# athas/raytracers

Hardware: AMD Instinct MI355X
Metric: Mray/s (primary+secondary) on rgbbox & irreg 1000x1000 (higher is better)
Workload: dtype f32

## Files before the change

raytracers_amd/csrc/api.cpp:

```cpp
#include <hip/hip_runtime.h>

#include <algorithm>
#include <chrono>
#include <cmath>
#include <cstdio>
#include <cstdlib>
#include <cstring>
#include <memory>
#include <string>
#include <vector>

#include "../../include/rt_mi355x.h"
#include "rt_device.hpp"
#include "rt_host.hpp"
#include "rt_internal.hpp"

namespace rti {
int fail(rt_context *ctx, const std::string &msg) {
  if (ctx) ctx->err = msg;
  return 1;
}
int hip_fail(rt_context *ctx, hipError_t e, const char *what) {
  return fail(ctx, std::string(what) + ": " + hipGetErrorString(e));
}
// ... 388 lines not shown
bool rt_scene_exceeds_l2(const rt_prepared *ps) { return static_cast<int64_t>(ps->n) * 80 > (int64_t(32) << 20); }

void set_cull(const rt_context *ctx, const rt_prepared *ps, const Plan &pl, const float *cams_dev, rtk::KParams *p) {
  if (ctx->cull == 0 || !ps->cull.ok || pl.variant != RT_VARIANT_POOLED || (pl.waves != 16 && pl.waves != 4)) return;
  if (ctx->cull < 0 && pl.lds_nodes == p->n_nodes && pl.lds_sph == p->n_sph) return;
  if (cams_dev == nullptr ? !rt::cull_origin_ok(ps->cull, &p->cam.ox) : (cams_dev != ctx->cams_dev || ctx->cams_host == nullptr)) return;
  for (int f = 0; cams_dev != nullptr && f < p->nframes; ++f)
    if (!rt::cull_origin_ok(ps->cull, ctx->cams_host + 12 * f)) return;
  p->cull = 1;
  p->cull_c2 = ps->cull.c2;
  p->cull_kappa = ps->cull.kappa;
}

void set_dark(const rt_context *ctx, bool instrumented, rtk::KParams *p) {
  p->dark = (ctx->dark_stop != 0 && p->cost == nullptr && (!instrumented || ctx->dark_stop > 0)) ? 1 : 0;
}

std::string pooled_launch_name(const rtk::KParams &p, int waves, int rays = 0) {
  rtk::PooledKey k{};
  return rtk::choose_pooled(p, false, waves, rays, &k) ? rtk::pooled_name(k) : "none";
}
const char *pooled_launch_nodes(const rtk::KParams &p, int waves) {
  rtk::PooledKey k{};
  return rtk::choose_pooled(p, false, waves, 0, &k) && rtk::pooled_presort(k) ? "sign-ordered" : "planes";
}

void frame_params(const rt_prepared *ps, int64_t h, int64_t w, int rows_per_tile, int part, int nparts, int max_depth, const float *cam12, rtk::KParams *p) {
  scene_params(ps, p);
  std::memcpy(&p->cam, cam12 ? static_cast<const void *>(cam12) : static_cast<const void *>(&ps->cam), sizeof(p->cam));
  p->w = static_cast<int>(w); p->h = static_cast<int>(h);
// ... 349 lines not shown
    RT_HIP(ctx, rtk::launch_persistent(p, false, pl.grid, pl.waves, ctx->stream));
    ctx->last_launch = "family=persistent";
    return 0;
  }
  if (ps->n >= (int64_t(1) << 22)) return fail(ctx, "pooled kernel: at most 2^22 spheres (work items and hit keys carry the leaf index in 22 bits)");
  if (p.rpt_log2 < 0) return fail(ctx, "pooled kernel: rows_per_tile must be a power of two");
  if (int rc = get_uv(ctx, w, h, &p.u_tab, &p.v_tab)) return rc;
  tick("uv tables");
  TileOrder *to = nullptr;
  if (ctx->adaptive_order && !p.cams)
    if (int rc = find_view(ctx, ps, p, pl, &to)) return rc;
  Tickets t;
  if (int rc = choose_tickets(ctx, ps, to, xq, tick, p, pl, &t)) return rc;
  set_cull(ctx, ps, pl, cams_dev, &p);
  set_dark(ctx, false, &p);
  tick("before launch");
  RT_HIP(ctx, rtk::launch_pooled(p, false, pl.grid, pl.waves, ctx->stream));
  tick("launch_pooled");
  char buf[256];
  std::snprintf(buf, sizeof buf, "family=pooled tickets=%s%s instantiation=%s frames=%d tiles=%d grid=%d waves=%d counters=%d%s deep_class=%d deep_split=%d recording=%d nodes=%s,dark=%d",
                p.px_hdr ? "pixel-list" : t.first_order ? "tiles-bit-reversed" : (p.order ? "tiles-ordered" : "tiles-raster"), t.borrowed ? "(borrowed)" : "",
                pooled_launch_name(p, pl.waves).c_str(), p.nframes, p.nchunks, pl.grid, pl.waves, p.nshards, p.interleave ? "(turns)" : "", p.px_hdr ? 0 : p.deep_class,
                p.px_hdr ? 0 : p.deep_split, p.cost ? (p.cost_px ? 2 : 1) : 0, pooled_launch_nodes(p, pl.waves), p.dark);
  ctx->last_launch = buf;
  if (to && p.cost) {
    to->sort_pending = true;
    to->sort_px = p.cost_px != nullptr;
    to->rec_out_skip = p.out_skip;
    if (ctx->eager_sort && (stream_was_idle || ctx->sync_policy))
      if (int rc = sort_view(ctx, ps, to, p, pl)) return rc;
    tick("record: eager sorts");
  }
  return 0;
}
using rti::enqueue_render;

extern "C" void rt_context_destroy(rt_context *ctx);

// ... 221 lines not shown
    ctx->px_solo_div = std::max(1, std::min(4096, v));
  } else if (k == "eager_sort") {
    drain_streams(ctx);
    ctx->eager_sort = v != 0;
  } else if (k == "borrow") {
    ctx->borrow = std::max(0, std::min(4, v));
  } else if (k == "stack_cap") {
    if (v != 0 && v != rtk::kSpillCapbTest) return fail(ctx, "stack_cap must be 0 or 192");
    ctx->stack_cap = v;
  } else if (k == "wide_waves") {
    ctx->wide_waves = std::max(0, std::min(2, v));
  } else if (k == "cull") {
    ctx->cull = std::max(-1, std::min(1, v));
  } else if (k == "dark_stop") {
    ctx->dark_stop = std::max(-1, std::min(1, v));
  } else if (k == "sync_policy") {
    ctx->sync_policy = v != 0;
  } else {
    return fail(ctx, "unknown option: " + k);
  }
  return 0;
}

extern "C" int rt_context_device_info(const rt_context *ctx, int *device, int *num_cu, int *lds_bytes, char *name,
                                      int name_len) {
  RT_LOCK(const_cast<rt_context *>(ctx));
  if (!ctx) return 1;
  if (device) *device = ctx->device;
  if (num_cu) *num_cu = ctx->num_cu;
  if (lds_bytes) *lds_bytes = ctx->lds_bytes;
// ... 66 lines not shown
  ps->bmax = reinterpret_cast<float *>(b + o_bmax); ps->left = reinterpret_cast<int32_t *>(b + o_left);
  ps->right = reinterpret_cast<int32_t *>(b + o_right); ps->parent = reinterpret_cast<int32_t *>(b + o_parent);
  ps->nodes = reinterpret_cast<float4 *>(b + o_nodes); ps->nodes64 = reinterpret_cast<float4 *>(b + o_nodes64);
  ps->sph = reinterpret_cast<float4 *>(b + o_sph); ps->col = reinterpret_cast<float4 *>(b + o_col);
  ps->ids = reinterpret_cast<int32_t *>(b + o_ids);
  return hipSuccess;
}

int host_build_upload(rt_context *ctx, rt_prepared *ps, const std::vector<rt::Sphere> &spheres, hipError_t *e) {
  const size_t n = spheres.size(), ni = n - 1;
  int rc = 0;
  auto put = [&](void *dst, const void *src, size_t bytes) {
    if (!rc && hipMemcpyAsync(dst, src, bytes, hipMemcpyHostToDevice, ctx->stream) != hipSuccess) rc = fail(ctx, "hipMemcpyAsync failed");
  };
  const rt::Lbvh bvh = rt::build_lbvh(spheres);
  const rt::TravLayout tl = rt::make_trav_layout(bvh, ctx->treelet);
  ps->height = tl.height;
  ps->tl_depth = tl.treelet_depth;
  put(ps->L7, bvh.L.data(), n * sizeof(rt::Sphere));
  put(ps->bmin, bvh.bmin.data(), ni * 3 * sizeof(float));
  put(ps->bmax, bvh.bmax.data(), ni * 3 * sizeof(float));
  put(ps->left, bvh.left.data(), ni * sizeof(int32_t));
  put(ps->right, bvh.right.data(), ni * sizeof(int32_t));
  put(ps->parent, bvh.parent.data(), ni * sizeof(int32_t));
  put(ps->nodes, tl.nodes.data(), ni * sizeof(rt::TravNode));
  put(ps->nodes64, tl.nodes64.data(), ni * 64);
  std::copy(tl.root_lo, tl.root_lo + 3, ps->root_lo);
  std::copy(tl.root_hi, tl.root_hi + 3, ps->root_hi);
  put(ps->sph, tl.sph.data(), n * 16);
  put(ps->col, tl.col.data(), n * 16);
  put(ps->ids, bvh.ids.data(), n * sizeof(int32_t));
// ... 7 lines not shown
  if (!ctx || !out || !scene) return fail(ctx, "null argument");
  if (h <= 0 || w <= 0) return fail(ctx, "image size must be positive");
  if (scene->desc.spheres.size() < 2) return fail(ctx, "scene needs at least 2 spheres");
  RT_HIP(ctx, hipSetDevice(ctx->device));
  (void)hipGetLastError();
  auto ps = std::make_unique<rt_prepared>();
  const size_t n = scene->desc.spheres.size();
  ps->n = static_cast<int64_t>(n);
  ps->home = ctx;
  ps->h = h; ps->w = w;
  ps->cam = rt::scene_camera(scene->desc, h, w);
  int rc = 0;
  hipError_t e = hipSuccess;
  RT_HIP(ctx, alloc_prepared_block(ctx, ps.get()));
  if (ctx->group) rti::group_prepare_begin(ctx, ps.get(), h, w, scene);
  if (ctx->gpu_build) {
    float *scene_dev = nullptr;
    {
      std::lock_guard<std::mutex> lock(scene->mu);
      for (const auto &c : scene->copies)
        if (c.device == ctx->device) scene_dev = c.p;
    }
    if (!scene_dev) {
      const size_t sbytes = n * sizeof(rt::Sphere);
      float *fresh = nullptr;
      e = hipMalloc(reinterpret_cast<void **>(&fresh), sbytes + 16);
      if (e == hipSuccess) {
        if (sbytes + 16 <= kStageBytes) {
          std::memcpy(ctx->stage, scene->desc.spheres.data(), sbytes);
          e = rtk::gpu_copy_from_pinned(fresh, ctx->stage, sbytes, ctx->stream);
// ... 10 lines not shown
          scene->copies.push_back({ctx->device, fresh});
          scene_dev = fresh;
          fresh = nullptr;
        }
      }
      if (fresh) (void)hipFree(fresh);
    }
    size_t tmp_bytes = rtk::gpu_build_scratch_bytes(static_cast<int>(n));
    char *tmp = nullptr;
    if (e == hipSuccess) e = pool_alloc(ctx, &tmp, &tmp_bytes);
    if (e == hipSuccess) {
      rtk::GpuBvhOut o{ps->L7, ps->bmin, ps->bmax, ps->left, ps->right, ps->parent, ps->nodes, ps->nodes64, ps->sph, ps->col, ps->ids};
      e = rtk::gpu_build_bvh(scene_dev, static_cast<int>(n), o, tmp, ctx->pinned, ctx->stream, &ps->height, ps->root_lo,
                             ps->root_hi);
      ps->tl_depth = rtk::kTreeletDepth;
    }
    if (tmp) {
      (void)hipStreamSynchronize(ctx->stream);
      pool_free(ctx, tmp, tmp_bytes);
    }
  } else {
    rc = host_build_upload(ctx, ps.get(), scene->desc.spheres, &e);
  }
  if (!rc && e == hipSuccess) {
    std::lock_guard<std::mutex> lock(scene->mu);
    if (!scene->cull_done) {
      scene->cull = rt::cull_scene_constants(scene->desc.spheres, 0);
      scene->cull_done = true;
    }
    ps->cull = scene->cull;
    ps->cull.ok = ps->cull.ok && ps->height <= static_cast<int>(log2f(static_cast<float>(n))) + 2;
  }
  if (!rc && e == hipSuccess && ctx->wide_waves != 0 && ps->height > 15 && n < (int64_t(1) << 22)) rc = ensure_spill(ctx, 64 * (ps->height + 2));
  const int grc = ctx->group ? rti::group_prepare_end(ctx, ps.get()) : 0;
  if (rc || e != hipSuccess) {
    rt_prepared_free(ctx, ps.release());
    return rc ? rc : hip_fail(ctx, e, "rt_prepare_scene");
  }
  if (grc) {
    rt_prepared_free(ctx, ps.release());
    return grc;
  }
  *out = ps.release();
  return 0;
// ... 39 lines not shown
      ps->tl_depth = rtk::kTreeletDepth;
    }
    (void)hipStreamSynchronize(ctx->stream);
    pool_free(ctx, tmp, tmp_bytes);
    if (*e != hipSuccess) return 0;
    rt::CullStats st;
    for (int a = 0; a < 3; ++a) {
      st.lo[a] = slot->lo[a];
      st.hi[a] = slot->hi[a];
    }
    st.r_min = slot->r_min;
    st.r_max = slot->r_max;
    st.c_max = slot->c_max;
    st.bad = slot->bad != 0;
    ps->cull = rt::cull_finish(st, n, 0);
  } else {
    std::vector<rt::Sphere> host(n);
    *e = hipMemcpyAsync(host.data(), spheres7_dev, n * sizeof(rt::Sphere), hipMemcpyDeviceToHost, ctx->stream);
    if (*e == hipSuccess) *e = hipStreamSynchronize(ctx->stream);
    if (*e != hipSuccess) return 0;
    if (int rc = host_build_upload(ctx, ps, host, e)) return rc;
    if (*e != hipSuccess) return 0;
    ps->cull = rt::cull_scene_constants(host, 0);
  }
  ps->cull.ok = ps->cull.ok && ps->height <= static_cast<int>(log2f(static_cast<float>(n))) + 2;
  if (ctx->wide_waves != 0 && ps->height > 15 && n < (size_t(1) << 22)) return ensure_spill(ctx, 64 * (ps->height + 2));
  return 0;
}

int device_spheres_ok(rt_context *ctx, const float *spheres7_dev, int64_t n) {
  if (!spheres7_dev) return fail(ctx, "null argument");
  if (n < 2 || n > (int64_t(1) << rtk::kMaxSpheresLog2)) return fail(ctx, "scene needs 2 .. 2^26 spheres");
  if (ctx->group) return fail(ctx, "device spheres: a multi-device context is not supported (use a context on one device)");
  return 0;
}

void reset_views(rt_context *ctx, rt_prepared *ps) {
  drain_streams(ctx);
// ... 324 lines not shown
        p.deep_split = dp.deep_split;
        p.deep_cap_log2 = dp.cap_log2;
        if (dp.sparse && ctx->grid_div == 0) pl.grid = pl.grid_full;
        if (px_list_launch(ctx, p, pl, &o)) {
          p.px_list = o.px_list;
          p.px_hdr = reinterpret_cast<const int *>(o.px_list + o.px_elems);
          p.px_hold = ctx->px_hold;
          p.px_prio = ctx->px_prio;
          p.solo = (ctx->trace_solo && o.px_solo && ctx->solo && ps->tl_depth == rtk::kTreeletDepth) ? 1 : 0;
          if (ctx->grid_div == 0 && pl.grid != pl.grid_full && counters_follow(&p, xq, pl.grid_full)) pl.grid = pl.grid_full;
        }
      }
    nw = pl.grid * pl.waves;
    set_cull(ctx, ps, pl, nullptr, &p);
    set_dark(ctx, true, &p);
    e = rtk::launch_pooled(p, true, pl.grid, pl.waves, ctx->stream);
    if (e == hipSuccess) e = hipStreamSynchronize(ctx->stream);
    if (e == hipSuccess) e = hipMemcpy(records, trace, sizeof(unsigned long long) * rtk::kTraceWords * static_cast<size_t>(nw), hipMemcpyDeviceToHost);
  }
  (void)hipFree(tmp);
  (void)hipFree(trace);
  if (rc) return rc;
  if (e != hipSuccess) return hip_fail(ctx, e, "rt_render_trace");
  *num_waves = nw;
  return 0;
}

extern "C" int rt_render_timed(rt_context *ctx, const rt_prepared *ps, int64_t h, int64_t w, int32_t max_depth,
                               int32_t rows_per_tile, int32_t part, int32_t nparts, int32_t *out_dev, int32_t warmup,
                               int32_t iters, float *ms_out) {
// ... 57 lines not shown
```

raytracers_amd/csrc/bvh_build.hip:

```cpp
#include <hip/hip_runtime.h>
#include <cstdio>
#include <cstring>
#include <cstdlib>

#include <cmath>
#include <cstdint>

#include "rt_device.hpp"
#include "treelet.h"

namespace rtk {
namespace {

constexpr int kBT = 256;
constexpr int kSortE = 4;
constexpr int kSortTile = kBT * kSortE;
constexpr int kSortBits = 4, kSortDigits = 1 << kSortBits, kSortWords = kSortDigits / 4;
constexpr int kRankMaxN = 24576;

__device__ __forceinline__ float f_min(float a, float b) { return fminf(a, b); }
__device__ __forceinline__ float f_max(float a, float b) { return fmaxf(a, b); }

__device__ __forceinline__ void sphere_centre(const float *s, float c[3]) {
  const float r = s[6];
// ... 1505 lines not shown
  if (threadIdx.x == 0) cull_acc_store(partial[blockIdx.x], a);
}
__global__ __launch_bounds__(kBT) void cull_stats_final_kernel(const CullStatsDev *__restrict__ partial, int nblocks, CullStatsDev *out) {
  CullAcc a;
  cull_acc_init(a);
  for (int b = threadIdx.x; b < nblocks; b += kBT) {
    CullAcc p;
    cull_acc_load(p, partial[b]);
    cull_acc_merge(a, p);
  }
  cull_acc_block(a);
  if (threadIdx.x == 0) cull_acc_store(*out, a);
}
}

hipError_t launch_cull_stats(const float *sph7_dev, int n, CullStatsDev *partial, CullStatsDev *out, hipStream_t st) {
  const int nb = cdiv(n, kBT), blocks = nb < kCullStatsBlocks ? nb : kCullStatsBlocks;
  if (blocks < 1) return hipErrorInvalidValue;
  hipLaunchKernelGGL(cull_stats_kernel, dim3(blocks), dim3(kBT), 0, st, sph7_dev, n, partial);
  hipLaunchKernelGGL(cull_stats_final_kernel, dim3(1), dim3(kBT), 0, st, (const CullStatsDev *)partial, blocks, out);
  return hipGetLastError();
}

__device__ __forceinline__ int fo_bitrev(int i, int bits) {
  int r = 0;
  for (int b = 0; b < bits; ++b) r |= ((i >> b) & 1) << (bits - 1 - b);
  return r;
}
__global__ __launch_bounds__(256) void first_order_rank_kernel(int tiles_x, int tiles_y, int *rank) {
  __shared__ unsigned short s_rev[1024];
// ... 51 lines not shown
```

raytracers_amd/csrc/host_build.cpp:

```cpp
#include "rt_host.hpp"

#include <algorithm>
#include <cmath>
#include <cstring>
#include <limits>
#include <numeric>

namespace rt {
namespace {

struct V3 {
  float x, y, z;
};
inline V3 operator+(V3 a, V3 b) { return {a.x + b.x, a.y + b.y, a.z + b.z}; }
inline V3 operator-(V3 a, V3 b) { return {a.x - b.x, a.y - b.y, a.z - b.z}; }
inline V3 operator*(float s, V3 v) { return {s * v.x, s * v.y, s * v.z}; }
inline float dot3(V3 a, V3 b) {
  float px = a.x * b.x, py = a.y * b.y, pz = a.z * b.z;
  return (px + py) + pz;
}
inline V3 unit(V3 v) { return (1.0f / std::sqrt(dot3(v, v))) * v; }
inline V3 cross3(V3 a, V3 b) {
  return {a.y * b.z - a.z * b.y, a.z * b.x - a.x * b.z, a.x * b.y - a.y * b.x};
}
// ... 363 lines not shown
  for (int a = 0; a < 3; ++a) {
    c.centre[a] = 0.5 * (s.lo[a] + s.hi[a]);
    diag2 += (s.hi[a] - s.lo[a]) * (s.hi[a] - s.lo[a]);
  }
  c.reach = 0.5 * std::sqrt(diag2) * (1.0 + 0x1p-20) + r_max;
  c.r_min = r_min;
  if (2.0 * c.reach > 0x1p15 * r_min) return c;
  const double c2 = 1.01 * (0x1p-16 / r_min + 0x1p-21);
  const double c0 = 1.01 * (0x1p-16 * r_max * r_max / r_min + 0x1p-18 * r_max + 0x1p-24 * c_max + 0x1p-21);
  c.c2 = std::nextafter(static_cast<float>(c2), INFINITY);
  c.kappa = std::nextafter(static_cast<float>(c0 / (c2 * 0.015625)), INFINITY);
  c.ok = std::isfinite(c.c2) && std::isfinite(c.kappa);
  return c;
}

bool cull_origin_ok(const CullConst &c, const float origin[3]) {
  if (!c.ok) return false;
  double d2 = 0.0;
  for (int a = 0; a < 3; ++a) {
    if (!std::isfinite(origin[a])) return false;
    d2 += (origin[a] - c.centre[a]) * (origin[a] - c.centre[a]);
  }
  return std::sqrt(d2) * (1.0 + 0x1p-20) + c.reach <= 0x1p15 * c.r_min;
}

}
```

raytracers_amd/csrc/lane_core.h:

```cpp
#pragma once
#include <math.h>
#include <stdint.h>

#if defined(__HIPCC__)
#define RT_HD __host__ __device__ __forceinline__
#else
#define RT_HD inline
#endif

namespace rtk {

constexpr float kTMax = 1000000000.0f;
constexpr float kEps = 0.1f;
constexpr float kNoHit = __builtin_inff();

struct Cam {
  float ox, oy, oz, lx, ly, lz, hx, hy, hz, vx, vy, vz;
};

struct Ray {
  float ox, oy, oz;
  float dx, dy, dz;
  float ix, iy, iz;
  float a;
// ... 76 lines not shown
}
RT_HD bool box_hit_clamped(const Ray &r, float lox, float loy, float loz, float hix, float hiy, float hiz, float tclamp) {
  return box_hit_interval(r, lox, loy, loz, hix, hiy, hiz, 0.0f, tclamp);
}
RT_HD bool box_hit(const Ray &r, float lox, float loy, float loz, float hix, float hiy, float hiz) {
  return box_hit_clamped(r, lox, loy, loz, hix, hiy, hiz, kTMax);
}

constexpr float kCullALo = 1.0f / 64.0f, kCullAHi = 1048576.0f;
RT_HD float cull_weight(const Ray &r, float c2) {
  const float m = fmaxf(fmaxf(fabsf(r.ix), fabsf(r.iy)), fabsf(r.iz));
  return (r.a >= kCullALo && r.a <= kCullAHi) ? m * r.a * c2 : kNoHit;
}
RT_HD float cull_limit(float best, float w2, float kappa) {
  return fminf(__builtin_fmaf(w2, __builtin_fmaf(best, best, kappa), best), kTMax);
}

RT_HD float sphere_root(const Ray &r, float px, float py, float pz, float rad) {
  const float ocx = r.ox - px, ocy = r.oy - py, ocz = r.oz - pz;
  const float b = dot3(ocx, ocy, ocz, r.dx, r.dy, r.dz);
  const float c = dot3(ocx, ocy, ocz, ocx, ocy, ocz) - rad * rad;
  const float disc = b * b - r.a * c;
  if (disc <= 0.0f) return kNoHit;
  const float sq = sqrtf(disc);
  float t = (-b - sq) / r.a;
  if (!(t > kEps)) {
    t = (-b + sq) / r.a;
    if (!(t > kEps)) return kNoHit;
  }
  return t;
// ... 128 lines not shown
```

raytracers_amd/csrc/render_kernels.hip:

```cpp
#include <hip/hip_runtime.h>

#include <mutex>
#include <type_traits>
#include <utility>

#include "lane_core.h"
#include "rt_device.hpp"
#include "treelet.h"

#ifdef RT_ISA_MARKS
#define RT_MARK(name) asm volatile("; RT_MARK " name)
#else
#define RT_MARK(name)
#endif

namespace rtk {

__device__ __forceinline__ int global_row(const KParams &p, int lrow) {
  const int k = lrow / p.rows_per_tile;
  return (k * p.nparts + p.part) * p.rows_per_tile + (lrow - k * p.rows_per_tile);
}

__device__ __forceinline__ size_t out_index(const KParams &p, int lrow, int col) {
  return (size_t)lrow * p.w + col + (size_t)(lrow / p.rows_per_tile) * (size_t)p.out_skip;
// ... 436 lines not shown
        if (pp->cost != nullptr) {
          if (pp->cost_px != nullptr) pp->cost_px[pix] = (unsigned char)(depth < 254 ? depth + 1 : 255);
          if (depth >= 2) atomicMax(&pp->cost[ptile], depth + 1);
        }
      }
      trace_flush();
      return;
    }
  }
}

__device__ __forceinline__ int launch_dark() {
  return *reinterpret_cast<const volatile __attribute__((address_space(4))) int *>(&((KParamsArg)__builtin_amdgcn_kernarg_segment_ptr())->dark);
}

template <int THREADS, bool ALL_LDS, bool STATS, bool SOLO, int TAIL = 0, bool ORD = false, bool CULL = false, int SPILL = 0, int RAYS = 0>
__global__ __launch_bounds__(THREADS, THREADS == 256 ? 5 : (THREADS / 64 + 3) / 4) void pooled_kernel(KParams p) {
  constexpr bool COLD = TAIL == 1, DONATE = TAIL == 2;
  constexpr bool ANY = RAYS == kRaysAny;
  static_assert(!RAYS || (!STATS && !SOLO && TAIL == 0 && !ORD && !CULL), "RAYS: the plain instantiations only");
  static_assert(!ORD || TAIL != 1, "ORD: no COLD variant");
  static_assert(!CULL || !ALL_LDS, "CULL: instantiated for the general scene path only");
  constexpr bool PRESORT = pooled_presort(ALL_LDS, SOLO, TAIL, ORD, RAYS);
  extern __shared__ float4 smem[];
  const int lane = threadIdx.x & 63;
  const int wave = threadIdx.x >> 6;
  const int plane = p.lds_nodes;
  const int sph_base = 4 * plane;
  const int per_wave_dw = pooled_wave_dw(p.ray_planes, p.capb, p.capl);
  unsigned *const wbase = reinterpret_cast<unsigned *>(smem + sph_base + p.lds_sph) + wave * per_wave_dw;
  unsigned long long *const wkey = reinterpret_cast<unsigned long long *>(wbase);
  int *const wcnt = reinterpret_cast<int *>(wbase + 128);
  unsigned *const wdump = wbase + 192;
  float4 *const wray = reinterpret_cast<float4 *>(wbase + kPooledWaveFixedDw);
  unsigned *const wbox = wbase + kPooledWaveFixedDw + 256 * p.ray_planes;
  unsigned *const wleaf = wbox + p.capb;
  const __amdgpu_buffer_rsrc_t rs_nodes = make_rsrc(p.nodes64, (unsigned)p.n_nodes * 64u);
  const __amdgpu_buffer_rsrc_t rs_sph = make_rsrc(p.sph, (unsigned)p.n_sph * 16u);
// ... 535 lines not shown
          }
        }
        asm volatile("" ::"v"(q2.w), "v"(q3.w), "v"(ra.w), "v"(ri.w));
        cl8 = f2i(q0.w); cr8 = f2i(q1.w);
        float limc = kTMax, limlo = 0.0f;
        if constexpr (CULL) limc = cull_limit(__uint_as_float(*reinterpret_cast<const unsigned *>(reinterpret_cast<const char *>(wkey) + 2 * sl4 + 4)), ri.w, p.cull_kappa);
        if constexpr (ANY) {
          limlo = ri.w;
          limc = __uint_as_float(*reinterpret_cast<const unsigned *>(reinterpret_cast<const char *>(wkey) + 2 * sl4 + 4));
        }
        m_hl = bal(box_hit_interval(q, q0.x, q0.y, q0.z, q1.x, q1.y, q1.z, limlo, limc));
        m_hr = bal(box_hit_interval(q, q2.x, q2.y, q2.z, q3.x, q3.y, q3.z, limlo, limc));
        }
        const unsigned long long m_ln = bal(cl8 < 0), m_rn = bal(cr8 < 0);
        const unsigned long long m_inl = m_act & ~m_ln & m_hl, m_inr = m_act & ~m_rn & m_hr;
        const unsigned long long m_lfl = m_act & m_ln, m_lfr = m_act & m_rn;
        if (STATS) n_box += __popcll(m_act & ~m_ln & (1ull << lane)) + __popcll(m_act & ~m_rn & (1ull << lane));
        const int c_inl = __popcll(m_inl), c_lfl = __popcll(m_lfl);
        const int dump = (int)(size_t)(wdump);
        const int b_box = (int)(size_t)(wbox + nbox), b_leaf = (int)(size_t)(wleaf + nleaf);
        const int a_l = sel_mask(m_lfl, sel_mask(m_inl, dump, b_box + 4 * lane_rank(m_inl)), b_leaf + 4 * lane_rank(m_lfl));
        const int a_r = sel_mask(m_lfr, sel_mask(m_inr, dump, b_box + 4 * lane_rank_from(m_inr, c_inl)),
                                 b_leaf + 4 * lane_rank_from(m_lfr, c_lfl));
        const unsigned low = PRESORT ? item & kPsItemLow : (unsigned)sl4;
        lds_store(a_l, (unsigned)cl8 | low);
        lds_store(a_r, (unsigned)cr8 | low);
        nbox = uni(nbox + c_inl + __popcll(m_inr));
        nleaf = uni(nleaf + c_lfl + __popcll(m_lfr));
        const unsigned long long m_two = m_inl & m_inr, m_none = m_act & ~(m_inl | m_inr);
        lds_add_masked(m_two | m_none, (int)(size_t)wcnt + sl4, sel_mask(m_two, -1, 1));
        if constexpr (FULL) RT_MARK("BOXFULL_END"); else RT_MARK("BOXPART_END");
// ... 2 lines not shown
        RT_MARK("BOX2_BEGIN");
        if (STATS) { tr_ops[0]++; tr_items[0] += nbox; }
        const int role = lane & 1;
        const int top = nbox - 1 - (lane >> 1);
        const unsigned item = wbox[top < 0 ? 0 : top];
        const bool act = top >= 0;
        nbox = uni(0);
        const int sl4 = (int)(item & 0xfcu);
        const int ni16 = (int)((item >> 4) & 0xfffffff0u);
        const float4 *const rayp = reinterpret_cast<const float4 *>(reinterpret_cast<const char *>(wray) + 4 * sl4);
        const float4 ra = rayp[0], ri = rayp[64];
        Ray q;
        q.ox = ra.x; q.oy = ra.y; q.oz = ra.z;
        q.ix = ri.x; q.iy = ri.y; q.iz = ri.z;
        int ref, cl8, cr8;
        bool pass, child_leaf;
        unsigned long long m_pass, m_cleaf, m_hl, m_hr;
        if constexpr (PRESORT) {
          const int sn = (int)(item >> 5), tx = sn & (int)kSignX, ty = sn & (int)kSignY, tz = sn & (int)kSignZ;
          const lds_cp cell = lds_ptr((unsigned)(size_t)smem + (item >> kPsItemShift) + 4u * (unsigned)role);
          const float cnx = lds_load4f(RT_PS_NEAR(cell, tx, kPsX)), cfx = lds_load4f(RT_PS_FAR(cell, tx, kPsX, kSignX));
          const float cny = lds_load4f(RT_PS_NEAR(cell, ty, kPsY)), cfy = lds_load4f(RT_PS_FAR(cell, ty, kPsY, kSignY));
          const float cnz = lds_load4f(RT_PS_NEAR(cell, tz, kPsZ)), cfz = lds_load4f(RT_PS_FAR(cell, tz, kPsZ, kSignZ));
          ref = f2i(lds_load4f(cell + kPsRefs));
          child_leaf = act & (ref < 0);
          pass = act & (ref >= 0) && box_hit_presorted(q, cnx, cfx, cny, cfy, cnz, cfz, 0.0f, kTMax);
          const lds_cp cell2 = lds_ptr((unsigned)(size_t)smem + (pass ? (unsigned)ref >> kPsItemShift : 0u));
          const v2f nx = lds_load8(RT_PS_NEAR(cell2, tx, kPsX)), fx = lds_load8(RT_PS_FAR(cell2, tx, kPsX, kSignX));
          const v2f ny = lds_load8(RT_PS_NEAR(cell2, ty, kPsY)), fy = lds_load8(RT_PS_FAR(cell2, ty, kPsY, kSignY));
          const v2f nz = lds_load8(RT_PS_NEAR(cell2, tz, kPsZ)), fz = lds_load8(RT_PS_FAR(cell2, tz, kPsZ, kSignZ));
          const v2f refs = lds_load8(cell2 + kPsRefs);
          asm volatile("" ::"v"(ra.w), "v"(ri.w));
          cl8 = f2i(refs.x); cr8 = f2i(refs.y);
          m_pass = bal(pass); m_cleaf = bal(child_leaf);
          m_hl = bal(box_hit_presorted(q, nx.x, fx.x, ny.x, fy.x, nz.x, fz.x, 0.0f, kTMax));
          m_hr = bal(box_hit_presorted(q, nx.y, fx.y, ny.y, fy.y, nz.y, fz.y, 0.0f, kTMax));
        } else {
        float4 lo, hi;
        {
          const bool res = ALL_LDS || ni16 < 16 * plane;
          const int lo16 = res ? ni16 : 0;
// ... 2 lines not shown
          hi = *reinterpret_cast<const float4 *>(np + (32 * role + 16) * plane);
          ref = f2i(reinterpret_cast<const float4 *>(np + 16 * role * plane)->w);
          if (!ALL_LDS && !res) {
            lo = buf_load16(rs_nodes, ni16 * 4 + 32 * role);
            hi = buf_load16(rs_nodes, ni16 * 4 + 32 * role + 16);
            ref = f2i(buf_load16(rs_nodes, ni16 * 4 + 16 * role).w);
          }
        }
        float limc = kTMax, limlo = 0.0f;
        if constexpr (CULL) limc = cull_limit(__uint_as_float(*reinterpret_cast<const unsigned *>(reinterpret_cast<const char *>(wkey) + 2 * sl4 + 4)), ri.w, p.cull_kappa);
        if constexpr (ANY) {
          limlo = ri.w;
          limc = __uint_as_float(*reinterpret_cast<const unsigned *>(reinterpret_cast<const char *>(wkey) + 2 * sl4 + 4));
        }
        child_leaf = act & (ref < 0);
        pass = act & (ref >= 0) && box_hit_interval(q, lo.x, lo.y, lo.z, hi.x, hi.y, hi.z, limlo, limc);
        if (STATS) n_box += (act & (ref >= 0)) ? 1 : 0;
        const int ci16 = pass ? (int)(((unsigned)ref >> 4) & 0xfffffff0u) : 0;
        float4 q0, q1, q2, q3;
        {
          const int lo16 = ALL_LDS ? ci16 : (ci16 < 16 * plane ? ci16 : 0);
          const float4 *const np = reinterpret_cast<const float4 *>(reinterpret_cast<const char *>(smem) + lo16);
          q0 = np[0]; q1 = np[plane]; q2 = np[2 * plane]; q3 = np[3 * plane];
          if (!ALL_LDS && ci16 >= 16 * plane) {
            q0 = buf_load16(rs_nodes, ci16 * 4);
            q1 = buf_load16(rs_nodes, ci16 * 4 + 16);
            q2 = buf_load16(rs_nodes, ci16 * 4 + 32);
            q3 = buf_load16(rs_nodes, ci16 * 4 + 48);
          }
        }
        asm volatile("" ::"v"(q2.w), "v"(q3.w), "v"(ra.w), "v"(ri.w), "v"(lo.w), "v"(hi.w));
        cl8 = f2i(q0.w); cr8 = f2i(q1.w);
        m_pass = bal(pass); m_cleaf = bal(child_leaf);
        m_hl = bal(box_hit_interval(q, q0.x, q0.y, q0.z, q1.x, q1.y, q1.z, limlo, limc));
        m_hr = bal(box_hit_interval(q, q2.x, q2.y, q2.z, q3.x, q3.y, q3.z, limlo, limc));
        }
        const unsigned long long m_ln = bal(cl8 < 0), m_rn = bal(cr8 < 0);
        const unsigned long long m_inl = m_pass & ~m_ln & m_hl, m_inr = m_pass & ~m_rn & m_hr;
        const unsigned long long m_lfl = (m_pass & m_ln) | m_cleaf, m_lfr = m_pass & m_rn;
        if (STATS) n_box += __popcll(m_pass & ~m_ln & (1ull << lane)) + __popcll(m_pass & ~m_rn & (1ull << lane));
        const int c_inl = __popcll(m_inl), c_lfl = __popcll(m_lfl);
        const int dump = (int)(size_t)(wdump);
        const int b_box = (int)(size_t)(wbox), b_leaf = (int)(size_t)(wleaf + nleaf);
        const int a_l = sel_mask(m_lfl, sel_mask(m_inl, dump, b_box + 4 * lane_rank(m_inl)), b_leaf + 4 * lane_rank(m_lfl));
        const int a_r = sel_mask(m_lfr, sel_mask(m_inr, dump, b_box + 4 * lane_rank_from(m_inr, c_inl)),
                                 b_leaf + 4 * lane_rank_from(m_lfr, c_lfl));
        const unsigned low = PRESORT ? item & kPsItemLow : (unsigned)sl4;
        lds_store(a_l, (unsigned)sel_mask(m_cleaf, cl8, ref) | low);
        lds_store(a_r, (unsigned)cr8 | low);
        nbox = uni(c_inl + __popcll(m_inr));
        nleaf = uni(nleaf + c_lfl + __popcll(m_lfr));
        const int d = sel_mask(m_inl, 0, 1) + sel_mask(m_inr, 0, 1) - sel_mask(bal(act & (role == 0)), 0, 1);
        lds_add_masked(bal(d != 0), (int)(size_t)wcnt + sl4, d);
        RT_MARK("BOX2_END");
// ... 525 lines not shown
```

raytracers_amd/csrc/rt_device.hpp:

```cpp
#pragma once
#include <hip/hip_runtime.h>
#include <stdint.h>

#include <string>

#include "lane_core.h"
#include "treelet.h"

namespace rtk {

constexpr int kTraceWords = 16;
constexpr int kStackPixel = 64;
constexpr int kPooledWaveFixedDw = 128 + 64 + 4;
constexpr int pooled_wave_dw(int ray_planes, int capb, int capl) { return kPooledWaveFixedDw + 256 * ray_planes + capb + capl; }
constexpr int kSpillCapb = 1088, kSpillCapbTest = 192;

constexpr int kQueueStride = 32;
constexpr int kMaxShards = 8;
constexpr int kQueueExit = kQueueStride * kMaxShards;
constexpr int kQueueDwords = kQueueStride * (kMaxShards + 1);
constexpr int kOrderTableDw = 16;
constexpr int order_table_ints(int ntiles) { return ntiles + kOrderTableDw * kMaxShards; }

struct Shard {
// ... 174 lines not shown
  int deep_cap_log2;
  int *cost;
  unsigned char *cost_px;
  const int *px_hdr;
  const unsigned *px_list;
  int px_hold;
  int px_prio;
  int cull;
  float cull_c2;
  float cull_kappa;
  int dark;
  const float *u_tab;
  const float *v_tab;
  unsigned *spill;
  int spill_stride;
  const float *rays;
  float *colour3;
  int nrays;
  unsigned char *occluded;
  float ray_tlo, ray_thi;
  const float *ray_tlo_dev, *ray_thi_dev;
};

#if defined(__HIPCC__)
__device__ __forceinline__ int f2i(float f) { return __float_as_int(f); }

typedef int v4i __attribute__((ext_vector_type(4)));
__device__ __forceinline__ __amdgpu_buffer_rsrc_t make_rsrc(const void *base, unsigned bytes) {
  return __builtin_amdgcn_make_buffer_rsrc(const_cast<void *>(base), 0, (int)bytes, 0x00020000);
}
// ... 75 lines not shown
    k.ord = true; k.solo = p.solo != 0; k.tail = p.donate ? 2 : 0;
    k.all_lds = all_lds && !k.cull;
  } else {
    k.solo = p.solo && p.nframes == 1 && p.order != nullptr && p.deep_class > 0 && p.deep_split == 6 && p.tl_log2 == kTreeletDepth;
    if (waves_per_wg == 16) k.tail = p.cold ? 1 : p.donate ? 2 : 0;
    else if (waves_per_wg != 4 && waves_per_wg != 8 && waves_per_wg != 12) return false;
    k.all_lds = all_lds && !k.cull;
  }
  *out = k;
  return true;
}

constexpr bool pooled_presort(bool all_lds, bool solo, int tail, bool ord, int rays) { return all_lds && !solo && tail == 0 && !ord && rays == 0; }
constexpr bool pooled_presort(const PooledKey &k) { return pooled_presort(k.all_lds, k.solo, k.tail, k.ord, k.rays); }

inline std::string pooled_name(const PooledKey &k) {
  std::string s = k.rays == kRaysAny ? "any" : k.ord ? "ORD" : k.tail == 1 ? "COLD" : k.tail == 2 ? "DONATE" : "";
  if (k.solo) s += s.empty() ? "SOLO" : "+SOLO";
  if (k.ord && k.tail == 2) s += "+DONATE";
  if (s.empty()) s = "plain";
  if (k.cull) s += "+CULL";
  if (k.spill) s += "+SPILL";
  return s;
}

hipError_t launch_pixel(const KParams &p, bool stats, hipStream_t stream);
hipError_t launch_pixel_rays(const KParams &p, hipStream_t stream);
hipError_t launch_persistent(const KParams &p, bool stats, int grid, int waves_per_wg, hipStream_t stream);
size_t persistent_lds_bytes(int lds_nodes, int lds_sph, int smax, int lmax, int waves_per_wg);
hipError_t launch_pooled(const KParams &p, bool stats, int grid, int waves_per_wg, hipStream_t stream, int rays = 0);
// ... 16 lines not shown
hipError_t gpu_build_bvh(const float *sph7_dev, int n, const GpuBvhOut &out, char *scratch, char *pinned, hipStream_t stream,
                         int *height_out, float root_lo[3], float root_hi[3]);
struct CullStatsDev {
  double c_max;
  float lo[3], hi[3];
  float r_min, r_max;
  int bad;
  int pad;
};
static_assert(sizeof(CullStatsDev) == 48, "CullStatsDev: 48 bytes");
constexpr size_t kCullStatsPinnedOffset = 256;
constexpr int kCullStatsBlocks = 1024;
constexpr size_t cull_stats_scratch_bytes() { return sizeof(CullStatsDev) * kCullStatsBlocks; }
hipError_t launch_cull_stats(const float *sph7_dev, int n, CullStatsDev *partial, CullStatsDev *out, hipStream_t stream);

constexpr int kOrderBlocksMax = 64;
constexpr int kOrderScratchInts = kMaxShards * 64 * kOrderBlocksMax;
hipError_t launch_tile_order(int *cost, int *order, int ntiles, int tiles_x, int nshards, int *scratch, hipStream_t stream);
struct PxGeom {
  int w, rows_local, rpt_log2, out_skip, tiles_x, tiles_y;
};
struct PxPolicy {
  int thr[kPxClasses - 1];
  int g[kPxClasses];
  int ray_ns;
  int nwaves;
  int solo_cap;
  int zip;
};
constexpr int kPxBlocksMax = 2048;
// ... 11 lines not shown
```

raytracers_amd/csrc/rt_host.hpp:

```cpp
#pragma once
#include <cmath>
#include <cstdint>
#include <string>
#include <vector>

#include "treelet.h"

namespace rt {

struct Sphere {
  float px, py, pz;
  float cr, cg, cb;
  float radius;
};
static_assert(sizeof(Sphere) == 28, "Sphere must be 7 packed floats");

struct SceneDesc {
  std::vector<Sphere> spheres;
  float look_from[3];
  float look_at[3];
  float fov;
};

struct Camera {
// ... 48 lines not shown
  float c2 = 0.0f, kappa = 0.0f;
  double centre[3] = {0, 0, 0}, reach = 0.0, r_min = 0.0;
};
CullConst cull_scene_constants(const std::vector<Sphere> &ts, int height);
struct CullStats {
  double lo[3] = {INFINITY, INFINITY, INFINITY}, hi[3] = {-INFINITY, -INFINITY, -INFINITY};
  double r_min = INFINITY, r_max = 0.0;
  double c_max = 0.0;
  bool bad = false;
};
CullStats cull_stats(const Sphere *ts, size_t n);
CullStats cull_stats_merge(const CullStats &a, const CullStats &b);
CullConst cull_finish(const CullStats &s, size_t n, int height);
bool cull_origin_ok(const CullConst &c, const float origin[3]);

int64_t part_rows(int64_t h, int32_t rows_per_tile, int32_t part, int32_t nparts);

}
```

raytracers_amd/csrc/rt_internal.hpp:

```cpp
#pragma once
#include <hip/hip_runtime.h>

#include <cstdint>
#include <future>
#include <mutex>
#include <string>
#include <vector>

#include "../../include/rt_mi355x.h"
#include "rt_device.hpp"
#include "rt_host.hpp"

struct rt_group;

struct rt_context {
  std::recursive_mutex mu;
  int device = 0;
  hipStream_t stream = nullptr;
  bool own_stream = false;
  std::string err;
  bool synced_since_render = true;
  std::string last_launch;
  int num_cu = 0;
  int lds_bytes = 0;
// ... 27 lines not shown
  int static_first = 1;
  int first_order = 1;
  int pixel_order = 1;
  int px_thr[4] = {0, 24, 14, 9};
  int px_g[5] = {0, 0, 0, 0, 0};
  int px_max_tiles = 40000;
  int px_ray_ns = 0;
  int px_hold = 0xf;
  int px_zip = 1;
  int px_prio = 3;
  int px_solo_div = 4;
  int stack_cap = 0;
  int wide_waves = 1;
  int cull = -1;
  int dark_stop = -1;
  int eager_sort = 1;
  int borrow = 1;
  int sync_policy = 0;
  hipStream_t sort_stream = nullptr, sort_stream_px = nullptr;
  hipEvent_t rec_event = nullptr;
  unsigned *queue_dev = nullptr;
  unsigned *spill_dev = nullptr;
  size_t spill_bytes = 0;
  int *order_scratch = nullptr;
  int *px_scratch = nullptr;
  char *within_scratch = nullptr;
  size_t within_bytes = 0;
  unsigned long long *stats_dev = nullptr;
  struct UvTable {
    int64_t w, h;
// ... 24 lines not shown
  unsigned long long class_chunks_used = 0;
  char *pinned = nullptr;
  char *stage = nullptr;
};

struct rt_scene {
  rt::SceneDesc desc;
  struct DevCopy {
    int device;
    float *p;
  };
  mutable std::mutex mu;
  mutable std::vector<DevCopy> copies;
  mutable bool cull_done = false;
  mutable rt::CullConst cull;
};

struct TileOrder {
  int64_t h, w;
  int32_t rows_per_tile, part, nparts, max_depth;
  float cam[12];
  int ntiles = 0;
  int nshards = 1;
  char *block = nullptr;
  size_t block_bytes = 0;
  rt_context *block_owner = nullptr;
  int *cost = nullptr;
  int *order = nullptr;
  bool valid = false;
  unsigned char *cost_px = nullptr;
// ... 14 lines not shown
};
constexpr int kClassSlotInts = 16, kClassSlots = 8;
constexpr int kClassChunks = 64;

struct rt_prepared {
  rt_context *home = nullptr;
  mutable std::recursive_mutex mu;
  mutable std::vector<TileOrder> orders;
  mutable uint64_t order_clock = 0;
  int64_t n = 0;
  int64_t h = 0, w = 0;
  rt::Camera cam{};
  int height = 0;
  int tl_depth = 1;
  rt::CullConst cull;
  float *L7 = nullptr, *bmin = nullptr, *bmax = nullptr;
  int32_t *left = nullptr, *right = nullptr, *parent = nullptr;
  float4 *nodes = nullptr, *nodes64 = nullptr, *sph = nullptr, *col = nullptr;
  int32_t *ids = nullptr;
  char *block = nullptr;
  size_t block_bytes = 0;
  float root_lo[3] = {0, 0, 0}, root_hi[3] = {0, 0, 0};
  int *classes_pinned = nullptr;
  int classes_chunk = -1;
  rt_context *classes_owner = nullptr;
  std::vector<rt_prepared *> replicas;
  std::vector<std::future<int>> replica_jobs;
};


// ... 56 lines not shown
```

Measured before the change: 20510.

## Add conservative leaf bounding boxes to cull sphere tests in pooled traversal

```diff
diff --git a/raytracers_amd/csrc/api.cpp b/raytracers_amd/csrc/api.cpp
--- a/raytracers_amd/csrc/api.cpp
+++ b/raytracers_amd/csrc/api.cpp
@@ -426,6 +426,18 @@
 
 void set_dark(const rt_context *ctx, bool instrumented, rtk::KParams *p) {
   p->dark = (ctx->dark_stop != 0 && p->cost == nullptr && (!instrumented || ctx->dark_stop > 0)) ? 1 : 0;
+}
+
+void set_leaf_box(const rt_context *ctx, const rt_prepared *ps, const Plan &pl, const float *cams_dev, bool instrumented, rtk::KParams *p) {
+  p->leaf_box = 0;
+  if (ctx->leaf_box == 0 || !ps->leaf.ok || pl.variant != RT_VARIANT_POOLED || (instrumented && ctx->leaf_box <= 0)) return;
+  if (pl.lds_nodes != p->n_nodes || pl.lds_sph != p->n_sph) return;
+  if (cams_dev == nullptr ? !rt::leaf_box_camera_ok(ps->leaf, &p->cam.ox) : (cams_dev != ctx->cams_dev || ctx->cams_host == nullptr)) return;
+  for (int f = 0; cams_dev != nullptr && f < p->nframes; ++f)
+    if (!rt::leaf_box_camera_ok(ps->leaf, ctx->cams_host + 12 * f)) return;
+  rtk::PooledKey k{};
+  if (!rtk::choose_pooled(*p, instrumented, pl.waves, 0, &k) || !rtk::pooled_leaf_box(k)) return;
+  p->leaf_box = 1;
 }
 
 std::string pooled_launch_name(const rtk::KParams &p, int waves, int rays = 0) {
@@ -805,14 +817,15 @@
   if (int rc = choose_tickets(ctx, ps, to, xq, tick, p, pl, &t)) return rc;
   set_cull(ctx, ps, pl, cams_dev, &p);
   set_dark(ctx, false, &p);
+  set_leaf_box(ctx, ps, pl, cams_dev, false, &p);
   tick("before launch");
   RT_HIP(ctx, rtk::launch_pooled(p, false, pl.grid, pl.waves, ctx->stream));
   tick("launch_pooled");
-  char buf[256];
-  std::snprintf(buf, sizeof buf, "family=pooled tickets=%s%s instantiation=%s frames=%d tiles=%d grid=%d waves=%d counters=%d%s deep_class=%d deep_split=%d recording=%d nodes=%s,dark=%d",
+  char buf[320];
+  std::snprintf(buf, sizeof buf, "family=pooled tickets=%s%s instantiation=%s frames=%d tiles=%d grid=%d waves=%d counters=%d%s deep_class=%d deep_split=%d recording=%d nodes=%s,dark=%d,leaf_box=%d",
                 p.px_hdr ? "pixel-list" : t.first_order ? "tiles-bit-reversed" : (p.order ? "tiles-ordered" : "tiles-raster"), t.borrowed ? "(borrowed)" : "",
                 pooled_launch_name(p, pl.waves).c_str(), p.nframes, p.nchunks, pl.grid, pl.waves, p.nshards, p.interleave ? "(turns)" : "", p.px_hdr ? 0 : p.deep_class,
-                p.px_hdr ? 0 : p.deep_split, p.cost ? (p.cost_px ? 2 : 1) : 0, pooled_launch_nodes(p, pl.waves), p.dark);
+                p.px_hdr ? 0 : p.deep_split, p.cost ? (p.cost_px ? 2 : 1) : 0, pooled_launch_nodes(p, pl.waves), p.dark, p.leaf_box);
   ctx->last_launch = buf;
   if (to && p.cost) {
     to->sort_pending = true;
@@ -1064,6 +1077,8 @@
     ctx->cull = std::max(-1, std::min(1, v));
   } else if (k == "dark_stop") {
     ctx->dark_stop = std::max(-1, std::min(1, v));
+  } else if (k == "leaf_box") {
+    ctx->leaf_box = std::max(-1, std::min(1, v));
   } else if (k == "sync_policy") {
     ctx->sync_policy = v != 0;
   } else {
@@ -1160,7 +1175,8 @@
     if (!rc && hipMemcpyAsync(dst, src, bytes, hipMemcpyHostToDevice, ctx->stream) != hipSuccess) rc = fail(ctx, "hipMemcpyAsync failed");
   };
   const rt::Lbvh bvh = rt::build_lbvh(spheres);
-  const rt::TravLayout tl = rt::make_trav_layout(bvh, ctx->treelet);
+  rt::TravLayout tl = rt::make_trav_layout(bvh, ctx->treelet);
+  rt::fill_leaf_boxes(tl, ps->leaf);
   ps->height = tl.height;
   ps->tl_depth = tl.treelet_depth;
   put(ps->L7, bvh.L.data(), n * sizeof(rt::Sphere));
@@ -1198,6 +1214,16 @@
   hipError_t e = hipSuccess;
   RT_HIP(ctx, alloc_prepared_block(ctx, ps.get()));
   if (ctx->group) rti::group_prepare_begin(ctx, ps.get(), h, w, scene);
+  {
+    std::lock_guard<std::mutex> lock(scene->mu);
+    if (!scene->cull_done) {
+      const rt::CullStats st = rt::cull_stats(scene->desc.spheres.data(), n);
+      scene->cull = rt::cull_finish(st, n, 0);
+      scene->leaf = rt::leaf_box_finish(st, n);
+      scene->cull_done = true;
+    }
+    ps->leaf = scene->leaf;
+  }
   if (ctx->gpu_build) {
     float *scene_dev = nullptr;
     {
@@ -1238,6 +1264,8 @@
       e = rtk::gpu_build_bvh(scene_dev, static_cast<int>(n), o, tmp, ctx->pinned, ctx->stream, &ps->height, ps->root_lo,
                              ps->root_hi);
       ps->tl_depth = rtk::kTreeletDepth;
+      if (e == hipSuccess && ps->leaf.ok)
+        e = rtk::launch_leaf_boxes(ps->nodes64, ps->sph, static_cast<int>(n) - 1, ps->leaf.q, ps->leaf.lin, ps->leaf.abs, ctx->stream);
     }
     if (tmp) {
       (void)hipStreamSynchronize(ctx->stream);
@@ -1248,10 +1276,6 @@
   }
   if (!rc && e == hipSuccess) {
     std::lock_guard<std::mutex> lock(scene->mu);
-    if (!scene->cull_done) {
-      scene->cull = rt::cull_scene_constants(scene->desc.spheres, 0);
-      scene->cull_done = true;
-    }
     ps->cull = scene->cull;
     ps->cull.ok = ps->cull.ok && ps->height <= static_cast<int>(log2f(static_cast<float>(n))) + 2;
   }
@@ -1321,14 +1345,22 @@
     st.c_max = slot->c_max;
     st.bad = slot->bad != 0;
     ps->cull = rt::cull_finish(st, n, 0);
+    ps->leaf = rt::leaf_box_finish(st, n);
+    if (ps->leaf.ok) {
+      *e = rtk::launch_leaf_boxes(ps->nodes64, ps->sph, static_cast<int>(n) - 1, ps->leaf.q, ps->leaf.lin, ps->leaf.abs, ctx->stream);
+      if (*e == hipSuccess) *e = hipStreamSynchronize(ctx->stream);
+      if (*e != hipSuccess) return 0;
+    }
   } else {
     std::vector<rt::Sphere> host(n);
     *e = hipMemcpyAsync(host.data(), spheres7_dev, n * sizeof(rt::Sphere), hipMemcpyDeviceToHost, ctx->stream);
     if (*e == hipSuccess) *e = hipStreamSynchronize(ctx->stream);
     if (*e != hipSuccess) return 0;
+    const rt::CullStats st = rt::cull_stats(host.data(), n);
+    ps->leaf = rt::leaf_box_finish(st, n);
     if (int rc = host_build_upload(ctx, ps, host, e)) return rc;
     if (*e != hipSuccess) return 0;
-    ps->cull = rt::cull_scene_constants(host, 0);
+    ps->cull = rt::cull_finish(st, n, 0);
   }
   ps->cull.ok = ps->cull.ok && ps->height <= static_cast<int>(log2f(static_cast<float>(n))) + 2;
   if (ctx->wide_waves != 0 && ps->height > 15 && n < (size_t(1) << 22)) return ensure_spill(ctx, 64 * (ps->height + 2));
@@ -1683,6 +1715,7 @@
     nw = pl.grid * pl.waves;
     set_cull(ctx, ps, pl, nullptr, &p);
     set_dark(ctx, true, &p);
+    set_leaf_box(ctx, ps, pl, nullptr, true, &p);
     e = rtk::launch_pooled(p, true, pl.grid, pl.waves, ctx->stream);
     if (e == hipSuccess) e = hipStreamSynchronize(ctx->stream);
     if (e == hipSuccess) e = hipMemcpy(records, trace, sizeof(unsigned long long) * rtk::kTraceWords * static_cast<size_t>(nw), hipMemcpyDeviceToHost);
diff --git a/raytracers_amd/csrc/bvh_build.hip b/raytracers_amd/csrc/bvh_build.hip
--- a/raytracers_amd/csrc/bvh_build.hip
+++ b/raytracers_amd/csrc/bvh_build.hip
@@ -1543,6 +1543,31 @@
 }
 }
 
+namespace {
+__global__ __launch_bounds__(kBT) void leaf_boxes_kernel(float4 *nodes64, const float4 *__restrict__ sph, int ni, float q, float lin, float abs) {
+  const int t = blockIdx.x * kBT + threadIdx.x;
+  if (t >= ni) return;
+#pragma unroll
+  for (int k = 0; k < 2; ++k) {
+    const int ref8 = __float_as_int(nodes64[4 * (size_t)t + k].w);
+    if (ref8 >= 0) continue;
+    const float4 s = sph[~(ref8 >> 8)];
+    float lo[3], hi[3];
+    leaf_box_bounds(s.x, s.y, s.z, s.w, q, lin, abs, lo, hi);
+    float4 *const slot = nodes64 + 4 * (size_t)t + 2 * k;
+    const float w0 = slot[0].w, w1 = slot[1].w;
+    slot[0] = make_float4(lo[0], lo[1], lo[2], w0);
+    slot[1] = make_float4(hi[0], hi[1], hi[2], w1);
+  }
+}
+}
+
+hipError_t launch_leaf_boxes(float4 *nodes64, const float4 *sph, int n_nodes, float q, float lin, float abs, hipStream_t st) {
+  if (n_nodes < 1) return hipErrorInvalidValue;
+  hipLaunchKernelGGL(leaf_boxes_kernel, dim3(cdiv(n_nodes, kBT)), dim3(kBT), 0, st, nodes64, sph, n_nodes, q, lin, abs);
+  return hipGetLastError();
+}
+
 hipError_t launch_cull_stats(const float *sph7_dev, int n, CullStatsDev *partial, CullStatsDev *out, hipStream_t st) {
   const int nb = cdiv(n, kBT), blocks = nb < kCullStatsBlocks ? nb : kCullStatsBlocks;
   if (blocks < 1) return hipErrorInvalidValue;
diff --git a/raytracers_amd/csrc/host_build.cpp b/raytracers_amd/csrc/host_build.cpp
--- a/raytracers_amd/csrc/host_build.cpp
+++ b/raytracers_amd/csrc/host_build.cpp
@@ -1,4 +1,5 @@
 #include "rt_host.hpp"
+#include "lane_core.h"
 
 #include <algorithm>
 #include <cmath>
@@ -401,6 +402,63 @@
   return c;
 }
 
+LeafBoxConst leaf_box_finish(const CullStats &s, size_t n) {
+  LeafBoxConst c;
+  if (n < 2 || s.bad) return c;
+  const double r_min = s.r_min, r_max = s.r_max, c_max = s.c_max;
+  if (c_max > 0x1p40) return c;
+  double diag2 = 0.0;
+  for (int a = 0; a < 3; ++a) {
+    c.centre[a] = 0.5 * (s.lo[a] + s.hi[a]);
+    diag2 += (s.hi[a] - s.lo[a]) * (s.hi[a] - s.lo[a]);
+  }
+  const double R = 0.5 * std::sqrt(diag2) * (1.0 + 0x1p-20);
+  c.d_eps = 2.0 * (R + r_max);
+  c.cam_max = c.d_eps - R;
+  if (c_max + c.d_eps > 0x1p15 * r_min) return c;
+  if (0x1p-18 * (c.d_eps * c.d_eps / (r_min * r_min) + 1.0) > 0.4375 * (1.0 - 0x1p-10)) return c;
+  c.q = std::nextafter(static_cast<float>(1.01 * 0x1p-19 * c.d_eps * c.d_eps), INFINITY);
+  c.lin = std::nextafter(static_cast<float>(1.01 * (0x1p-19 + 0x1p-21)), INFINITY);
+  c.abs = std::nextafter(static_cast<float>(1.01 * 0x1p-22 * (c.d_eps + c_max)), INFINITY);
+  c.ok = std::isfinite(c.q) && std::isfinite(c.abs) && c.q > 0.0f;
+  return c;
+}
+
+bool leaf_box_camera_ok(const LeafBoxConst &c, const float cam12[12]) {
+  if (!c.ok) return false;
+  double m = 0.0;
+  for (int i = 0; i < 12; ++i) {
+    if (!std::isfinite(cam12[i])) return false;
+    m = std::max(m, std::fabs(static_cast<double>(cam12[i])));
+  }
+  if (m > 0x1p15) return false;
+  const double o[3] = {cam12[0], cam12[1], cam12[2]}, l[3] = {cam12[3] - o[0], cam12[4] - o[1], cam12[5] - o[2]};
+  const double hv[3] = {cam12[6], cam12[7], cam12[8]}, vv[3] = {cam12[9], cam12[10], cam12[11]};
+  double d2 = 0.0;
+  for (int a = 0; a < 3; ++a) d2 += (o[a] - c.centre[a]) * (o[a] - c.centre[a]);
+  if (!(std::sqrt(d2) * (1.0 + 0x1p-20) <= c.cam_max)) return false;
+  const double nx = hv[1] * vv[2] - hv[2] * vv[1], ny = hv[2] * vv[0] - hv[0] * vv[2], nz = hv[0] * vv[1] - hv[1] * vv[0];
+  const double nn = std::sqrt(nx * nx + ny * ny + nz * nz);
+  if (!(nn > 0.0)) return false;
+  const double plane = std::fabs(l[0] * nx + l[1] * ny + l[2] * nz) / nn;
+  return plane * (1.0 - 0x1p-20) - 0x1p-19 * m >= 0x1p-12;
+}
+
+void fill_leaf_boxes(TravLayout &t, const LeafBoxConst &c) {
+  if (!c.ok) return;
+  const size_t ni = t.nodes64.size() / 16;
+  for (size_t ti = 0; ti < ni; ++ti) {
+    float *q = &t.nodes64[16 * ti];
+    for (int k = 0; k < 2; ++k) {
+      int32_t ref8;
+      std::memcpy(&ref8, &q[3 + 4 * k], 4);
+      if (ref8 >= 0) continue;
+      const float *s = &t.sph[4 * static_cast<size_t>(~(ref8 >> 8))];
+      rtk::leaf_box_bounds(s[0], s[1], s[2], s[3], c.q, c.lin, c.abs, &q[8 * k], &q[8 * k + 4]);
+    }
+  }
+}
+
 bool cull_origin_ok(const CullConst &c, const float origin[3]) {
   if (!c.ok) return false;
   double d2 = 0.0;
diff --git a/raytracers_amd/csrc/lane_core.h b/raytracers_amd/csrc/lane_core.h
--- a/raytracers_amd/csrc/lane_core.h
+++ b/raytracers_amd/csrc/lane_core.h
@@ -114,6 +114,13 @@
 }
 RT_HD float cull_limit(float best, float w2, float kappa) {
   return fminf(__builtin_fmaf(w2, __builtin_fmaf(best, best, kappa), best), kTMax);
+}
+
+RT_HD float leaf_box_eps(float rad, float q, float lin, float abs) { return (q / rad + lin * rad) + abs; }
+RT_HD void leaf_box_bounds(float px, float py, float pz, float rad, float q, float lin, float abs, float lo[3], float hi[3]) {
+  const float rw = rad + leaf_box_eps(rad, q, lin, abs);
+  lo[0] = px - rw; lo[1] = py - rw; lo[2] = pz - rw;
+  hi[0] = px + rw; hi[1] = py + rw; hi[2] = pz + rw;
 }
 
 RT_HD float sphere_root(const Ray &r, float px, float py, float pz, float rad) {
diff --git a/raytracers_amd/csrc/render_kernels.hip b/raytracers_amd/csrc/render_kernels.hip
--- a/raytracers_amd/csrc/render_kernels.hip
+++ b/raytracers_amd/csrc/render_kernels.hip
@@ -474,6 +474,12 @@
   return *reinterpret_cast<const volatile __attribute__((address_space(4))) int *>(&((KParamsArg)__builtin_amdgcn_kernarg_segment_ptr())->dark);
 }
 
+__device__ __forceinline__ unsigned long long launch_leaf_off() {
+  KParamsArg kp = (KParamsArg)__builtin_amdgcn_kernarg_segment_ptr();
+  asm volatile("" : "+s"(kp));
+  return (unsigned long long)(unsigned)kp->leaf_box - 1ull;
+}
+
 template <int THREADS, bool ALL_LDS, bool STATS, bool SOLO, int TAIL = 0, bool ORD = false, bool CULL = false, int SPILL = 0, int RAYS = 0>
 __global__ __launch_bounds__(THREADS, THREADS == 256 ? 5 : (THREADS / 64 + 3) / 4) void pooled_kernel(KParams p) {
   constexpr bool COLD = TAIL == 1, DONATE = TAIL == 2;
@@ -482,6 +488,7 @@
   static_assert(!ORD || TAIL != 1, "ORD: no COLD variant");
   static_assert(!CULL || !ALL_LDS, "CULL: instantiated for the general scene path only");
   constexpr bool PRESORT = pooled_presort(ALL_LDS, SOLO, TAIL, ORD, RAYS);
+  constexpr bool LEAFBOX = pooled_leaf_box(THREADS, ALL_LDS, STATS, SOLO, CULL, RAYS);
   extern __shared__ float4 smem[];
   const int lane = threadIdx.x & 63;
   const int wave = threadIdx.x >> 6;
@@ -1047,7 +1054,8 @@
         }
         const unsigned long long m_ln = bal(cl8 < 0), m_rn = bal(cr8 < 0);
         const unsigned long long m_inl = m_act & ~m_ln & m_hl, m_inr = m_act & ~m_rn & m_hr;
-        const unsigned long long m_lfl = m_act & m_ln, m_lfr = m_act & m_rn;
+        const unsigned long long m_off = LEAFBOX ? launch_leaf_off() : ~0ull;
+        const unsigned long long m_lfl = m_act & m_ln & (m_hl | m_off), m_lfr = m_act & m_rn & (m_hr | m_off);
         if (STATS) n_box += __popcll(m_act & ~m_ln & (1ull << lane)) + __popcll(m_act & ~m_rn & (1ull << lane));
         const int c_inl = __popcll(m_inl), c_lfl = __popcll(m_lfl);
         const int dump = (int)(size_t)(wdump);
@@ -1080,7 +1088,7 @@
         q.ox = ra.x; q.oy = ra.y; q.oz = ra.z;
         q.ix = ri.x; q.iy = ri.y; q.iz = ri.z;
         int ref, cl8, cr8;
-        bool pass, child_leaf;
+        bool pass, child_leaf, own;
         unsigned long long m_pass, m_cleaf, m_hl, m_hr;
         if constexpr (PRESORT) {
           const int sn = (int)(item >> 5), tx = sn & (int)kSignX, ty = sn & (int)kSignY, tz = sn & (int)kSignZ;
@@ -1090,7 +1098,8 @@
           const float cnz = lds_load4f(RT_PS_NEAR(cell, tz, kPsZ)), cfz = lds_load4f(RT_PS_FAR(cell, tz, kPsZ, kSignZ));
           ref = f2i(lds_load4f(cell + kPsRefs));
           child_leaf = act & (ref < 0);
-          pass = act & (ref >= 0) && box_hit_presorted(q, cnx, cfx, cny, cfy, cnz, cfz, 0.0f, kTMax);
+          own = box_hit_presorted(q, cnx, cfx, cny, cfy, cnz, cfz, 0.0f, kTMax);
+          pass = act & (ref >= 0) & own;
           const lds_cp cell2 = lds_ptr((unsigned)(size_t)smem + (pass ? (unsigned)ref >> kPsItemShift : 0u));
           const v2f nx = lds_load8(RT_PS_NEAR(cell2, tx, kPsX)), fx = lds_load8(RT_PS_FAR(cell2, tx, kPsX, kSignX));
           const v2f ny = lds_load8(RT_PS_NEAR(cell2, ty, kPsY)), fy = lds_load8(RT_PS_FAR(cell2, ty, kPsY, kSignY));
@@ -1123,7 +1132,13 @@
           limc = __uint_as_float(*reinterpret_cast<const unsigned *>(reinterpret_cast<const char *>(wkey) + 2 * sl4 + 4));
         }
         child_leaf = act & (ref < 0);
-        pass = act & (ref >= 0) && box_hit_interval(q, lo.x, lo.y, lo.z, hi.x, hi.y, hi.z, limlo, limc);
+        if constexpr (!LEAFBOX) {
+          pass = act & (ref >= 0) && box_hit_interval(q, lo.x, lo.y, lo.z, hi.x, hi.y, hi.z, limlo, limc);
+          own = pass;
+        } else {
+          own = box_hit_interval(q, lo.x, lo.y, lo.z, hi.x, hi.y, hi.z, limlo, limc);
+          pass = act & (ref >= 0) & own;
+        }
         if (STATS) n_box += (act & (ref >= 0)) ? 1 : 0;
         const int ci16 = pass ? (int)(((unsigned)ref >> 4) & 0xfffffff0u) : 0;
         float4 q0, q1, q2, q3;
@@ -1146,7 +1161,8 @@
         }
         const unsigned long long m_ln = bal(cl8 < 0), m_rn = bal(cr8 < 0);
         const unsigned long long m_inl = m_pass & ~m_ln & m_hl, m_inr = m_pass & ~m_rn & m_hr;
-        const unsigned long long m_lfl = (m_pass & m_ln) | m_cleaf, m_lfr = m_pass & m_rn;
+        const unsigned long long m_off = LEAFBOX ? launch_leaf_off() : ~0ull, m_own = bal(own);
+        const unsigned long long m_lfl = (m_pass & m_ln & (m_hl | m_off)) | (m_cleaf & (m_own | m_off)), m_lfr = m_pass & m_rn & (m_hr | m_off);
         if (STATS) n_box += __popcll(m_pass & ~m_ln & (1ull << lane)) + __popcll(m_pass & ~m_rn & (1ull << lane));
         const int c_inl = __popcll(m_inl), c_lfl = __popcll(m_lfl);
         const int dump = (int)(size_t)(wdump);
diff --git a/raytracers_amd/csrc/rt_device.hpp b/raytracers_amd/csrc/rt_device.hpp
--- a/raytracers_amd/csrc/rt_device.hpp
+++ b/raytracers_amd/csrc/rt_device.hpp
@@ -212,6 +212,7 @@
   const float *v_tab;
   unsigned *spill;
   int spill_stride;
+  int leaf_box;
   const float *rays;
   float *colour3;
   int nrays;
@@ -317,6 +318,11 @@
 constexpr bool pooled_presort(bool all_lds, bool solo, int tail, bool ord, int rays) { return all_lds && !solo && tail == 0 && !ord && rays == 0; }
 constexpr bool pooled_presort(const PooledKey &k) { return pooled_presort(k.all_lds, k.solo, k.tail, k.ord, k.rays); }
 
+constexpr bool pooled_leaf_box(int threads, bool all_lds, bool stats, bool solo, bool cull, int rays) {
+  return rays == 0 && !cull && (stats || (all_lds && !(threads == 256 && solo)));
+}
+constexpr bool pooled_leaf_box(const PooledKey &k) { return pooled_leaf_box(k.threads, k.all_lds, k.stats, k.solo, k.cull, k.rays); }
+
 inline std::string pooled_name(const PooledKey &k) {
   std::string s = k.rays == kRaysAny ? "any" : k.ord ? "ORD" : k.tail == 1 ? "COLD" : k.tail == 2 ? "DONATE" : "";
   if (k.solo) s += s.empty() ? "SOLO" : "+SOLO";
@@ -363,6 +369,8 @@
 constexpr size_t cull_stats_scratch_bytes() { return sizeof(CullStatsDev) * kCullStatsBlocks; }
 hipError_t launch_cull_stats(const float *sph7_dev, int n, CullStatsDev *partial, CullStatsDev *out, hipStream_t stream);
 
+hipError_t launch_leaf_boxes(float4 *nodes64, const float4 *sph, int n_nodes, float q, float lin, float abs, hipStream_t stream);
+
 constexpr int kOrderBlocksMax = 64;
 constexpr int kOrderScratchInts = kMaxShards * 64 * kOrderBlocksMax;
 hipError_t launch_tile_order(int *cost, int *order, int ntiles, int tiles_x, int nshards, int *scratch, hipStream_t stream);
diff --git a/raytracers_amd/csrc/rt_host.hpp b/raytracers_amd/csrc/rt_host.hpp
--- a/raytracers_amd/csrc/rt_host.hpp
+++ b/raytracers_amd/csrc/rt_host.hpp
@@ -86,6 +86,15 @@
 CullConst cull_finish(const CullStats &s, size_t n, int height);
 bool cull_origin_ok(const CullConst &c, const float origin[3]);
 
+struct LeafBoxConst {
+  bool ok = false;
+  float q = 0.0f, lin = 0.0f, abs = 0.0f;
+  double centre[3] = {0, 0, 0}, d_eps = 0.0, cam_max = 0.0;
+};
+LeafBoxConst leaf_box_finish(const CullStats &s, size_t n);
+bool leaf_box_camera_ok(const LeafBoxConst &c, const float cam12[12]);
+void fill_leaf_boxes(TravLayout &t, const LeafBoxConst &c);
+
 int64_t part_rows(int64_t h, int32_t rows_per_tile, int32_t part, int32_t nparts);
 
 }
diff --git a/raytracers_amd/csrc/rt_internal.hpp b/raytracers_amd/csrc/rt_internal.hpp
--- a/raytracers_amd/csrc/rt_internal.hpp
+++ b/raytracers_amd/csrc/rt_internal.hpp
@@ -65,6 +65,7 @@
   int wide_waves = 1;
   int cull = -1;
   int dark_stop = -1;
+  int leaf_box = -1;
   int eager_sort = 1;
   int borrow = 1;
   int sync_policy = 0;
@@ -119,6 +120,7 @@
   mutable std::vector<DevCopy> copies;
   mutable bool cull_done = false;
   mutable rt::CullConst cull;
+  mutable rt::LeafBoxConst leaf;
 };
 
 struct TileOrder {
@@ -163,6 +165,7 @@
   int height = 0;
   int tl_depth = 1;
   rt::CullConst cull;
+  rt::LeafBoxConst leaf;
   float *L7 = nullptr, *bmin = nullptr, *bmax = nullptr;
   int32_t *left = nullptr, *right = nullptr, *parent = nullptr;
   float4 *nodes = nullptr, *nodes64 = nullptr, *sph = nullptr, *col = nullptr;
```

Result: faster. 21450, median of 6 (+4.6%).
